# ShadenSmith/splatt

Measured on NVIDIA H100. Metric: MTTKRP nnz*R/sec per mode, higher is better.
Workload: dtype f64

## Files before the change

### splatt_b200/csrc/mttkrp_tiled.cu

```cuda
#include "mttkrp_kernels.cuh"

namespace spb200 {

constexpr int kTW   = 24;
constexpr int kTRS  = 96;
constexpr int kTB   = 4;
constexpr int kSlab = 32;

struct TiledArgs {
  const SpRec *    rec;
  const uint32_t * rootid;
  const uint32_t * seg_off;
  const uint32_t * rroot;
  const double *   leaf;
  const double *   parent;
  double *         out;
  uint32_t         ntiles, tile_rows, leaf_rows;
  uint32_t         tile_bytes;
  uint32_t         tpitch;
  uint32_t         acc_rows;
  int              ldm, col0, col_end;
  int              whole;
};

__device__ __forceinline__ void mbar_wait(uint64_t * bar, uint32_t parity) {
  while (!mbar_try_wait(bar, parity)) {}
}

__device__ __forceinline__ void consumers_sync() {
  asm volatile("bar.sync 1, %0;" ::"n"(kTW * 32) : "memory");
}

template <int L>
__global__ void __launch_bounds__((kTW + 1) * 32, 1) mttkrp_tiled_root3(const TiledArgs a) {
  constexpr int G  = 32 / L;
  constexpr int NG = kTW * G;

  extern __shared__ __align__(128) unsigned char smem[];
  unsigned char * tiles = smem;
  double *   accs = reinterpret_cast<double *>(smem + 2 * a.tile_bytes);
  SpRec *    ring = reinterpret_cast<SpRec *>(accs + static_cast<size_t>(a.acc_rows) * kSlab);
  uint64_t * bars = reinterpret_cast<uint64_t *>(ring + kTW * 2 * kTRS);
  uint64_t * tile_full  = bars;
  uint64_t * tile_empty = bars + 2;
  uint64_t * rec_full   = bars + 4;

  const int      warp  = threadIdx.x >> 5;
  const int      lane  = threadIdx.x & 31;
  const uint32_t pitch = static_cast<uint32_t>(a.ldm) * 8u;
  const uint32_t NT    = a.ntiles;
  const uint32_t NS    = static_cast<uint32_t>(a.col_end - a.col0 + kSlab - 1) / kSlab;
  const uint32_t * so  = a.seg_off + static_cast<size_t>(blockIdx.x) * NT;
  const uint32_t r_lo  = a.rroot[2 * blockIdx.x];
  const uint32_t nrows = (a.rroot[2 * blockIdx.x + 1] >= r_lo) ? a.rroot[2 * blockIdx.x + 1] - r_lo + 1 : 0u;

  for (uint32_t i = threadIdx.x; i < nrows * (kSlab / 2); i += blockDim.x)
    reinterpret_cast<double2 *>(accs)[i] = make_double2(0.0, 0.0);
  if (threadIdx.x == 0) {
    for (int b = 0; b < 2; ++b) { mbar_init(&tile_full[b], 1); mbar_init(&tile_empty[b], kTW); }
    for (int w = 0; w < kTW * 2; ++w) mbar_init(&rec_full[w], 1);
    asm volatile("fence.mbarrier_init.release.cluster;" ::: "memory");
    asm volatile("fence.proxy.async.shared::cta;" ::: "memory");
  }
  __syncthreads();

  auto tile_rows_of = [&](uint32_t t) {
    const uint32_t first = t * a.tile_rows;
    return min(a.tile_rows, a.leaf_rows - first);
  };

  if (warp == kTW) {
    for (uint32_t gt = 0; gt < NS * NT; ++gt) {
      const uint32_t t = gt % NT, b = gt & 1u;
      if (gt >= 2) mbar_wait(&tile_empty[b], ((gt - 2) >> 1) & 1u);
      const uint32_t rows = tile_rows_of(t);
      unsigned char * dst = tiles + b * a.tile_bytes;
      if (a.whole) {
        if (lane == 0) {
          const uint32_t bytes = rows * pitch;
          mbar_arrive_expect_tx(&tile_full[b], bytes);
          const char * src = reinterpret_cast<const char *>(a.leaf) +
                             static_cast<size_t>(t) * a.tile_rows * pitch;
          for (uint32_t off = 0; off < bytes; off += 32768u)
            tma_bulk_g2s(dst + off, src + off, min(32768u, bytes - off), &tile_full[b]);
        }
      } else {
        const int      sc0 = a.col0 + static_cast<int>(gt / NT) * kSlab;
        const uint32_t sb  = static_cast<uint32_t>(min(kSlab, a.col_end - sc0)) * 8u;
        if (lane == 0) mbar_arrive_expect_tx(&tile_full[b], rows * sb);
        __syncwarp();
        const double * src = a.leaf + static_cast<size_t>(t) * a.tile_rows * a.ldm + sc0;
        for (uint32_t i = lane; i < rows; i += 32)
          tma_bulk_g2s(dst + i * a.tpitch, src + static_cast<size_t>(i) * a.ldm, sb, &tile_full[b]);
      }
    }
    return;
  }

  const int  grp    = lane / L;
  const int  gl     = lane % L;
  const bool leader = (gl == 0);
  SpRec *    myring = ring + warp * 2 * kTRS;
  uint64_t * mybars = rec_full + warp * 2;

  auto part = [&](uint32_t t, uint32_t g0, uint32_t g1, uint32_t & lo, uint32_t & hi) {
    const uint32_t s0 = so[t], len = so[t + 1] - s0;
    lo = s0 + static_cast<uint32_t>(static_cast<unsigned long long>(g0) * len / NG);
    hi = s0 + static_cast<uint32_t>(static_cast<unsigned long long>(g1) * len / NG);
  };

  uint32_t it = 0, ioff = 0, ij = 0;
  auto issue_next = [&]() {
    if (it >= NS * NT) return;
    uint32_t ws, we;
    part(it % NT, warp * G, (warp + 1) * G, ws, we);
    const uint32_t rs  = ws + ioff;
    const uint32_t cnt = (rs < we) ? min(static_cast<uint32_t>(kTRS), we - rs) : 0u;
    if (lane == 0) {
      uint64_t * bar = &mybars[ij & 1u];
      if (cnt) {
        asm volatile("fence.proxy.async.shared::cta;" ::: "memory");
        mbar_arrive_expect_tx(bar, cnt * 16u);
        tma_bulk_g2s(myring + (ij & 1u) * kTRS, a.rec + rs, cnt * 16u, bar);
      } else {
        mbar_arrive(bar);
      }
    }
    ++ij;
    ioff += kTRS;
    if (ws + ioff >= we) { ++it; ioff = 0; }
  };
  issue_next();
  issue_next();

  const double2 zero2 = make_double2(0.0, 0.0);
  double2 acc1 = zero2, acc0 = zero2;
  uint32_t j = 0;

  for (uint32_t s = 0; s < NS; ++s) {
    const int    sc0  = a.col0 + static_cast<int>(s) * kSlab;
    const int    sw   = min(kSlab, a.col_end - sc0);
    const bool   act  = (2 * gl) < sw;
    const int    c2   = act ? 2 * gl : 0;
    const char * pbase = reinterpret_cast<const char *>(a.parent + sc0 + c2);
    const uint32_t tcol = static_cast<uint32_t>((a.whole ? sc0 : 0) + c2) * 8u;
    double *     abase = accs + c2;
    auto flush = [&](uint32_t n) {
      double * p = abase + static_cast<size_t>(__ldg(&a.rootid[n]) - r_lo) * kSlab;
      atomicAdd(p, acc0.x);
      atomicAdd(p + 1, acc0.y);
      acc0 = zero2;
    };

    for (uint32_t t = 0; t < NT; ++t) {
      const uint32_t gt = s * NT + t;
      mbar_wait(&tile_full[gt & 1u], (gt >> 1) & 1u);
      const unsigned char * tile = tiles + (gt & 1u) * a.tile_bytes + tcol;
      const uint32_t kbase = t * a.tile_rows;
      uint32_t ws, we, gs, ge;
      part(t, warp * G, (warp + 1) * G, ws, we);
      part(t, warp * G + grp, warp * G + grp + 1, gs, ge);
      const uint32_t nr = (we > ws) ? (we - ws + kTRS - 1) / kTRS : 1u;
      for (uint32_t i = 0; i < nr; ++i, ++j) {
        mbar_wait(&mybars[j & 1u], (j >> 1) & 1u);
        SpRec *        buf = myring + (j & 1u) * kTRS;
        const uint32_t rs  = ws + i * kTRS;
        const uint32_t re  = min(we, rs + kTRS);
        const uint32_t lo  = max(gs, rs), hi = min(ge, re);
        if (leader && hi > lo && hi == ge)
          buf[hi - 1 - rs].aux = (buf[hi - 1 - rs].aux & SPB200_IDX_MASK) | (2u << SPB200_IDX_BITS);
        __syncwarp();
        if (act && hi > lo) {
          uint32_t n = lo;
          for (; n + kTB <= hi; n += kTB) {
            uint4   q[kTB];
            double2 b[kTB], r[kTB];
            uint32_t any = 0;
#pragma unroll
            for (int u = 0; u < kTB; ++u) {
              q[u] = *reinterpret_cast<const uint4 *>(&buf[n + u - rs]);
              any |= q[u].w;
            }
#pragma unroll
            for (int u = 0; u < kTB; ++u)
              if (q[u].w >> SPB200_IDX_BITS) r[u] = ld_row_na(pbase, q[u].w & SPB200_IDX_MASK, pitch);
#pragma unroll
            for (int u = 0; u < kTB; ++u)
              b[u] = *reinterpret_cast<const double2 *>(tile + static_cast<size_t>(q[u].z - kbase) * a.tpitch);
            if ((any >> (SPB200_IDX_BITS + 1)) == 0) {
#pragma unroll
              for (int u = 0; u < kTB; ++u) {
                const double v = __hiloint2double(static_cast<int>(q[u].y), static_cast<int>(q[u].x));
                acc1           = fma2(v, b[u], acc1);
                if (q[u].w >> SPB200_IDX_BITS) { acc0 = fma2(acc1, r[u], acc0); acc1 = zero2; }
              }
            } else {
#pragma unroll
              for (int u = 0; u < kTB; ++u) {
                const double   v = __hiloint2double(static_cast<int>(q[u].y), static_cast<int>(q[u].x));
                const uint32_t c = q[u].w >> SPB200_IDX_BITS;
                acc1             = fma2(v, b[u], acc1);
                if (c) {
                  acc0 = fma2(acc1, r[u], acc0);
                  acc1 = zero2;
                  if (c >= 2) flush(n + u);
                }
              }
            }
          }
          for (; n < hi; ++n) {
            const uint4    q = *reinterpret_cast<const uint4 *>(&buf[n - rs]);
            const double   v = __hiloint2double(static_cast<int>(q.y), static_cast<int>(q.x));
            const uint32_t c = q.w >> SPB200_IDX_BITS;
            const double2  b = *reinterpret_cast<const double2 *>(tile + static_cast<size_t>(q.z - kbase) * a.tpitch);
            acc1             = fma2(v, b, acc1);
            if (c) {
              acc0 = fma2(acc1, ld_row_na(pbase, q.w & SPB200_IDX_MASK, pitch), acc0);
              acc1 = zero2;
              if (c >= 2) flush(n);
            }
          }
        }
        __syncwarp();
        issue_next();
      }
      __syncwarp();
      if (lane == 0) mbar_arrive(&tile_empty[gt & 1u]);
    }

    consumers_sync();
    const uint32_t pairs = static_cast<uint32_t>(sw) / 2u;
    for (uint32_t i = threadIdx.x; i < nrows * pairs; i += kTW * 32) {
      const uint32_t row = i / pairs, c = 2u * (i % pairs);
      double2 *      src = reinterpret_cast<double2 *>(accs + static_cast<size_t>(row) * kSlab + c);
      const double2  v   = *src;
      *src = zero2;
      double * dst = a.out + static_cast<size_t>(r_lo + row) * a.ldm + sc0 + c;
      if (row == 0 || row + 1 == nrows) {
        atomicAdd(dst, v.x);
        atomicAdd(dst + 1, v.y);
      } else {
        *reinterpret_cast<double2 *>(dst) = v;
      }
    }
    consumers_sync();
  }
}

}

static size_t tiled_smem_bytes(uint32_t tile_rows, uint32_t acc_rows) {
  using namespace spb200;
  return (2 * (size_t)tile_rows + acc_rows) * kSlab * 8 + sizeof(SpRec) * kTW * 2 * kTRS +
         sizeof(uint64_t) * (4 + 2 * kTW) + 128;
}

uint32_t spb200_tiled_rows_for(uint32_t acc_rows) {
  const size_t fixed = tiled_smem_bytes(0, acc_rows);
  if (fixed >= 227 * 1024) return 0;
  return (uint32_t)((227 * 1024 - fixed) / 2 / (spb200::kSlab * 8));
}

bool spb200_tiled_applicable(const FiberStream & s, int kind) {
  return s.nmodes == 3 && kind == SPB200_KIND_ROOT && s.seg_off && s.rootid && s.rroot &&
         s.ntiles > 0 && tiled_smem_bytes(s.ktile_rows, s.acc_rows) <= 227 * 1024;
}

int spb200_launch_tiled_root3(const FiberStream & s, int ldm, int col_begin, int col_end,
                              const double * leaf, const double * parent, double * d_out,
                              cudaStream_t stream) {
  using namespace spb200;
  TiledArgs a;
  a.rec = s.rec; a.rootid = s.rootid; a.seg_off = s.seg_off; a.rroot = s.rroot;
  a.leaf = leaf; a.parent = parent; a.out = d_out;
  a.ntiles = s.ntiles; a.tile_rows = s.ktile_rows; a.leaf_rows = (uint32_t)s.leaf_rows;
  a.acc_rows = s.acc_rows;
  a.ldm = ldm; a.col0 = col_begin; a.col_end = col_end;
  a.whole = (col_end - col_begin <= kSlab && ldm <= kSlab) ? 1 : 0;
  a.tile_bytes = s.ktile_rows * kSlab * 8u;
  a.tpitch = a.whole ? (uint32_t)ldm * 8u : kSlab * 8u;
  const size_t smem = tiled_smem_bytes(s.ktile_rows, s.acc_rows);
  const int threads = (kTW + 1) * 32;
  const unsigned grid = s.kranges;
#define SPB200_TILED_LAUNCH(LL)                                                                   \
  do {                                                                                            \
    static bool set[64] = {false};                      \
    int dev_ = 0;                                                                                 \
    SPB200_CUDA_OK(cudaGetDevice(&dev_));                                                         \
    if (dev_ < 0 || dev_ >= 64 || !set[dev_]) {                                                   \
      SPB200_CUDA_OK(cudaFuncSetAttribute(mttkrp_tiled_root3<LL>,                                 \
                                          cudaFuncAttributeMaxDynamicSharedMemorySize, 227 * 1024)); \
      if (dev_ >= 0 && dev_ < 64) set[dev_] = true;                                               \
    }                                                                                             \
    mttkrp_tiled_root3<LL><<<grid, threads, smem, stream>>>(a);                                   \
  } while (0)
  const int width = col_end - col_begin;
  if (width <= 8) SPB200_TILED_LAUNCH(4);
  else if (width <= 16) SPB200_TILED_LAUNCH(8);
  else SPB200_TILED_LAUNCH(16);
#undef SPB200_TILED_LAUNCH
  spb200_count_launches(1);
  SPB200_CUDA_OK(cudaGetLastError());
  return SPLATT_SUCCESS;
}
```

Before: 604.4 billion.

## Remove dedicated producer warp; last-finishing consumer warp issues next tile load

```diff
diff --git a/splatt_b200/csrc/mttkrp_tiled.cu b/splatt_b200/csrc/mttkrp_tiled.cu
--- a/splatt_b200/csrc/mttkrp_tiled.cu
+++ b/splatt_b200/csrc/mttkrp_tiled.cu
@@ -27,12 +27,14 @@
   while (!mbar_try_wait(bar, parity)) {}
 }
 
-__device__ __forceinline__ void consumers_sync() {
-  asm volatile("bar.sync 1, %0;" ::"n"(kTW * 32) : "memory");
+__device__ __forceinline__ double2 lds_f64x2(uint32_t addr) {
+  double2 r;
+  asm volatile("ld.shared.v2.f64 {%0, %1}, [%2];" : "=d"(r.x), "=d"(r.y) : "r"(addr));
+  return r;
 }
 
 template <int L>
-__global__ void __launch_bounds__((kTW + 1) * 32, 1) mttkrp_tiled_root3(const TiledArgs a) {
+__global__ void __launch_bounds__(kTW * 32, 1) mttkrp_tiled_root3(const TiledArgs a) {
   constexpr int G  = 32 / L;
   constexpr int NG = kTW * G;
 
@@ -41,9 +43,9 @@
   double *   accs = reinterpret_cast<double *>(smem + 2 * a.tile_bytes);
   SpRec *    ring = reinterpret_cast<SpRec *>(accs + static_cast<size_t>(a.acc_rows) * kSlab);
   uint64_t * bars = reinterpret_cast<uint64_t *>(ring + kTW * 2 * kTRS);
-  uint64_t * tile_full  = bars;
-  uint64_t * tile_empty = bars + 2;
-  uint64_t * rec_full   = bars + 4;
+  uint64_t * tile_full = bars;
+  uint32_t * tile_left = reinterpret_cast<uint32_t *>(bars + 2);
+  uint64_t * rec_full  = bars + 4;
 
   const int      warp  = threadIdx.x >> 5;
   const int      lane  = threadIdx.x & 31;
@@ -52,49 +54,48 @@
   const uint32_t NS    = static_cast<uint32_t>(a.col_end - a.col0 + kSlab - 1) / kSlab;
   const uint32_t * so  = a.seg_off + static_cast<size_t>(blockIdx.x) * NT;
   const uint32_t r_lo  = a.rroot[2 * blockIdx.x];
-  const uint32_t nrows = (a.rroot[2 * blockIdx.x + 1] >= r_lo) ? a.rroot[2 * blockIdx.x + 1] - r_lo + 1 : 0u;
-
-  for (uint32_t i = threadIdx.x; i < nrows * (kSlab / 2); i += blockDim.x)
+  auto range_rows = [&]() {
+    const uint32_t r_hi = __ldg(&a.rroot[2 * blockIdx.x + 1]);
+    return (r_hi >= r_lo) ? r_hi - r_lo + 1 : 0u;
+  };
+
+  for (uint32_t i = threadIdx.x, nrows = range_rows(); i < nrows * (kSlab / 2); i += blockDim.x)
     reinterpret_cast<double2 *>(accs)[i] = make_double2(0.0, 0.0);
   if (threadIdx.x == 0) {
-    for (int b = 0; b < 2; ++b) { mbar_init(&tile_full[b], 1); mbar_init(&tile_empty[b], kTW); }
+    for (int b = 0; b < 2; ++b) { mbar_init(&tile_full[b], 1); tile_left[b] = 0; }
     for (int w = 0; w < kTW * 2; ++w) mbar_init(&rec_full[w], 1);
     asm volatile("fence.mbarrier_init.release.cluster;" ::: "memory");
     asm volatile("fence.proxy.async.shared::cta;" ::: "memory");
   }
   __syncthreads();
 
-  auto tile_rows_of = [&](uint32_t t) {
-    const uint32_t first = t * a.tile_rows;
-    return min(a.tile_rows, a.leaf_rows - first);
+  auto load_tile = [&](uint32_t gt) {
+    const uint32_t t = gt % NT, b = gt & 1u;
+    const uint32_t rows = min(a.tile_rows, a.leaf_rows - t * a.tile_rows);
+    unsigned char * dst = tiles + b * a.tile_bytes;
+    asm volatile("fence.proxy.async.shared::cta;" ::: "memory");
+    if (a.whole) {
+      if (lane == 0) {
+        const uint32_t bytes = rows * pitch;
+        mbar_arrive_expect_tx(&tile_full[b], bytes);
+        const char * src = reinterpret_cast<const char *>(a.leaf) +
+                           static_cast<size_t>(t) * a.tile_rows * pitch;
+        for (uint32_t off = 0; off < bytes; off += 32768u)
+          tma_bulk_g2s(dst + off, src + off, min(32768u, bytes - off), &tile_full[b]);
+      }
+    } else {
+      const int      sc0 = a.col0 + static_cast<int>(gt / NT) * kSlab;
+      const uint32_t sb  = static_cast<uint32_t>(min(kSlab, a.col_end - sc0)) * 8u;
+      if (lane == 0) mbar_arrive_expect_tx(&tile_full[b], rows * sb);
+      __syncwarp();
+      const double * src = a.leaf + static_cast<size_t>(t) * a.tile_rows * a.ldm + sc0;
+      for (uint32_t i = lane; i < rows; i += 32)
+        tma_bulk_g2s(dst + i * a.tpitch, src + static_cast<size_t>(i) * a.ldm, sb, &tile_full[b]);
+    }
   };
-
-  if (warp == kTW) {
-    for (uint32_t gt = 0; gt < NS * NT; ++gt) {
-      const uint32_t t = gt % NT, b = gt & 1u;
-      if (gt >= 2) mbar_wait(&tile_empty[b], ((gt - 2) >> 1) & 1u);
-      const uint32_t rows = tile_rows_of(t);
-      unsigned char * dst = tiles + b * a.tile_bytes;
-      if (a.whole) {
-        if (lane == 0) {
-          const uint32_t bytes = rows * pitch;
-          mbar_arrive_expect_tx(&tile_full[b], bytes);
-          const char * src = reinterpret_cast<const char *>(a.leaf) +
-                             static_cast<size_t>(t) * a.tile_rows * pitch;
-          for (uint32_t off = 0; off < bytes; off += 32768u)
-            tma_bulk_g2s(dst + off, src + off, min(32768u, bytes - off), &tile_full[b]);
-        }
-      } else {
-        const int      sc0 = a.col0 + static_cast<int>(gt / NT) * kSlab;
-        const uint32_t sb  = static_cast<uint32_t>(min(kSlab, a.col_end - sc0)) * 8u;
-        if (lane == 0) mbar_arrive_expect_tx(&tile_full[b], rows * sb);
-        __syncwarp();
-        const double * src = a.leaf + static_cast<size_t>(t) * a.tile_rows * a.ldm + sc0;
-        for (uint32_t i = lane; i < rows; i += 32)
-          tma_bulk_g2s(dst + i * a.tpitch, src + static_cast<size_t>(i) * a.ldm, sb, &tile_full[b]);
-      }
-    }
-    return;
+  if (warp == 0) {
+    load_tile(0);
+    if (NS * NT > 1) load_tile(1);
   }
 
   const int  grp    = lane / L;
@@ -109,8 +110,8 @@
     hi = s0 + static_cast<uint32_t>(static_cast<unsigned long long>(g1) * len / NG);
   };
 
-  uint32_t it = 0, ioff = 0, ij = 0;
-  auto issue_next = [&]() {
+  uint32_t it = 0, ioff = 0;
+  auto issue_next = [&](uint32_t ij) {
     if (it >= NS * NT) return;
     uint32_t ws, we;
     part(it % NT, warp * G, (warp + 1) * G, ws, we);
@@ -126,12 +127,11 @@
         mbar_arrive(bar);
       }
     }
-    ++ij;
     ioff += kTRS;
     if (ws + ioff >= we) { ++it; ioff = 0; }
   };
-  issue_next();
-  issue_next();
+  issue_next(0);
+  issue_next(1);
 
   const double2 zero2 = make_double2(0.0, 0.0);
   double2 acc1 = zero2, acc0 = zero2;
@@ -142,7 +142,7 @@
     const int    sw   = min(kSlab, a.col_end - sc0);
     const bool   act  = (2 * gl) < sw;
     const int    c2   = act ? 2 * gl : 0;
-    const char * pbase = reinterpret_cast<const char *>(a.parent + sc0 + c2);
+    const uint32_t poff = static_cast<uint32_t>(sc0 + c2) * 8u;
     const uint32_t tcol = static_cast<uint32_t>((a.whole ? sc0 : 0) + c2) * 8u;
     double *     abase = accs + c2;
     auto flush = [&](uint32_t n) {
@@ -154,19 +154,18 @@
 
     for (uint32_t t = 0; t < NT; ++t) {
       const uint32_t gt = s * NT + t;
-      mbar_wait(&tile_full[gt & 1u], (gt >> 1) & 1u);
-      const unsigned char * tile = tiles + (gt & 1u) * a.tile_bytes + tcol;
-      const uint32_t kbase = t * a.tile_rows;
+      const uint32_t tile = smem_u32(tiles) + (gt & 1u) * a.tile_bytes + tcol - t * a.tile_rows * a.tpitch;
       uint32_t ws, we, gs, ge;
       part(t, warp * G, (warp + 1) * G, ws, we);
       part(t, warp * G + grp, warp * G + grp + 1, gs, ge);
       const uint32_t nr = (we > ws) ? (we - ws + kTRS - 1) / kTRS : 1u;
       for (uint32_t i = 0; i < nr; ++i, ++j) {
         mbar_wait(&mybars[j & 1u], (j >> 1) & 1u);
-        SpRec *        buf = myring + (j & 1u) * kTRS;
         const uint32_t rs  = ws + i * kTRS;
         const uint32_t re  = min(we, rs + kTRS);
         const uint32_t lo  = max(gs, rs), hi = min(ge, re);
+        if (i == 0) mbar_wait(&tile_full[gt & 1u], (gt >> 1) & 1u);
+        SpRec *        buf = myring + (j & 1u) * kTRS;
         if (leader && hi > lo && hi == ge)
           buf[hi - 1 - rs].aux = (buf[hi - 1 - rs].aux & SPB200_IDX_MASK) | (2u << SPB200_IDX_BITS);
         __syncwarp();
@@ -183,10 +182,10 @@
             }
 #pragma unroll
             for (int u = 0; u < kTB; ++u)
-              if (q[u].w >> SPB200_IDX_BITS) r[u] = ld_row_na(pbase, q[u].w & SPB200_IDX_MASK, pitch);
+              b[u] = lds_f64x2(tile + q[u].z * a.tpitch);
 #pragma unroll
             for (int u = 0; u < kTB; ++u)
-              b[u] = *reinterpret_cast<const double2 *>(tile + static_cast<size_t>(q[u].z - kbase) * a.tpitch);
+              if (q[u].w >> SPB200_IDX_BITS) r[u] = ld_row_na(reinterpret_cast<const char *>(a.parent) + poff, q[u].w & SPB200_IDX_MASK, pitch);
             if ((any >> (SPB200_IDX_BITS + 1)) == 0) {
 #pragma unroll
               for (int u = 0; u < kTB; ++u) {
@@ -212,24 +211,31 @@
             const uint4    q = *reinterpret_cast<const uint4 *>(&buf[n - rs]);
             const double   v = __hiloint2double(static_cast<int>(q.y), static_cast<int>(q.x));
             const uint32_t c = q.w >> SPB200_IDX_BITS;
-            const double2  b = *reinterpret_cast<const double2 *>(tile + static_cast<size_t>(q.z - kbase) * a.tpitch);
+            const double2  b = lds_f64x2(tile + q.z * a.tpitch);
             acc1             = fma2(v, b, acc1);
             if (c) {
-              acc0 = fma2(acc1, ld_row_na(pbase, q.w & SPB200_IDX_MASK, pitch), acc0);
+              acc0 = fma2(acc1, ld_row_na(reinterpret_cast<const char *>(a.parent) + poff, q.w & SPB200_IDX_MASK, pitch), acc0);
               acc1 = zero2;
               if (c >= 2) flush(n);
             }
           }
         }
         __syncwarp();
-        issue_next();
+        issue_next(j + 2);
       }
       __syncwarp();
-      if (lane == 0) mbar_arrive(&tile_empty[gt & 1u]);
+      uint32_t last = 0;
+      if (lane == 0) {
+        __threadfence_block();
+        last = ((atomicAdd(&tile_left[gt & 1u], 1u) + 1u) % kTW == 0) ? 1u : 0u;
+        __threadfence_block();
+      }
+      if (__shfl_sync(0xffffffffu, last, 0) && gt + 2 < NS * NT) load_tile(gt + 2);
     }
 
-    consumers_sync();
+    __syncthreads();
     const uint32_t pairs = static_cast<uint32_t>(sw) / 2u;
+    const uint32_t nrows = range_rows();
     for (uint32_t i = threadIdx.x; i < nrows * pairs; i += kTW * 32) {
       const uint32_t row = i / pairs, c = 2u * (i % pairs);
       double2 *      src = reinterpret_cast<double2 *>(accs + static_cast<size_t>(row) * kSlab + c);
@@ -243,7 +249,7 @@
         *reinterpret_cast<double2 *>(dst) = v;
       }
     }
-    consumers_sync();
+    __syncthreads();
   }
 }
 
@@ -280,7 +286,7 @@
   a.tile_bytes = s.ktile_rows * kSlab * 8u;
   a.tpitch = a.whole ? (uint32_t)ldm * 8u : kSlab * 8u;
   const size_t smem = tiled_smem_bytes(s.ktile_rows, s.acc_rows);
-  const int threads = (kTW + 1) * 32;
+  const int threads = kTW * 32;
   const unsigned grid = s.kranges;
 #define SPB200_TILED_LAUNCH(LL)                                                                   \
   do {                                                                                            \
@@ -290,6 +296,9 @@
     if (dev_ < 0 || dev_ >= 64 || !set[dev_]) {                                                   \
       SPB200_CUDA_OK(cudaFuncSetAttribute(mttkrp_tiled_root3<LL>,                                 \
                                           cudaFuncAttributeMaxDynamicSharedMemorySize, 227 * 1024)); \
+      SPB200_CUDA_OK(cudaFuncSetAttribute(mttkrp_tiled_root3<LL>,                                 \
+                                          cudaFuncAttributePreferredSharedMemoryCarveout,         \
+                                          cudaSharedmemCarveoutMaxShared));                       \
       if (dev_ >= 0 && dev_ < 64) set[dev_] = true;                                               \
     }                                                                                             \
     mttkrp_tiled_root3<LL><<<grid, threads, smem, stream>>>(a);                                   \
```

New measurement: 656.4 billion (median of 6 runs). 8.6% higher.
